# JuliaLinearAlgebra/AlgebraicMultigrid.jl

Measured on AMD Instinct MI355X. Metric: V-cycle unknowns/sec + fine-level SpMV GB/s (% HBM peak), 3-D Poisson 256^3, higher is better.
Workload: dtype f64

## Files before the change

### algebraicmultigrid.jl_amd/_libs.py

```python
import ctypes as C
import os

_HERE = os.path.dirname(os.path.abspath(__file__))
SETUP_SO = os.path.join(_HERE, "libamgsetup.so")
HIP_SO = os.path.join(_HERE, "libamghip.so")
HIP_F32_SO = os.path.join(_HERE, "libamghip_f32.so")

i32p = C.POINTER(C.c_int32)
f64p = C.POINTER(C.c_double)
i64 = C.c_int64
vp = C.c_void_p


class AMGError(RuntimeError):
    pass


class amgs_options(C.Structure):
    _fields_ = [("theta", C.c_double), ("max_levels", C.c_int32), ("max_coarse", C.c_int32),
                ("hermitian", C.c_int32), ("sa_omega", C.c_double), ("sa_improve_iters", C.c_int32),
                ("sa_B_is_vector", C.c_int32)]


class amgh_smoother_t(C.Structure):
# ... 141 lines not shown
    L.amgh_dev_upload.argtypes = [C.c_int, vp, vp, i64]
    L.amgh_dev_download.argtypes = [C.c_int, vp, vp, i64]
    L.amgh_dev_sync.argtypes = [C.c_int]
    L.amgh_stream.restype = vp
    L.amgh_stream.argtypes = [vp]
    L.amgh_timer_begin.argtypes = [vp]
    L.amgh_timer_end.argtypes = [vp, C.POINTER(C.c_double)]
    L.amgh_bench_op.argtypes = [vp, C.c_int, C.c_int, C.c_int, C.c_int, C.POINTER(C.c_double)]
    L.amgh_debug_chain_timing.argtypes = [C.c_int, vp]
    L.amgh_debug_merged_sweep_host.argtypes = [i64, i64, vp, vp, vp, C.c_int, C.c_int, C.c_double, vp, vp]
    L.amgh_debug_bw_poll_giveups.argtypes = [vp, C.c_int]
    L.amgh_debug_bw_mode.argtypes = [vp, C.c_int]
    L.amgh_debug_bw_dict.argtypes = [vp, C.c_int]
    L.amgh_debug_bw_late.argtypes = [vp, C.c_int]
    L.amgh_debug_coded_ops.argtypes = [vp, C.c_int]
    L.amgh_debug_bw_sweep_host.argtypes = [i64, vp, vp, vp, C.c_int, C.c_int, C.c_double, vp, vp, vp]
    L.amgh_debug_bw_dict_sweep_host.argtypes = [i64, vp, vp, vp, C.c_int, C.c_int, vp, vp, vp]
    L.amgh_debug_set_tunable.argtypes = [C.c_char_p, C.c_int]
    L.amgh_debug_get_tunable.argtypes = [C.c_char_p, C.POINTER(C.c_int)]
    L.amgh_profile_enable.argtypes = [vp, C.c_int]
    L.amgh_profile_read.argtypes = [vp, vp, C.c_int]
    L.amgh_set_use_graph.argtypes = [vp, C.c_int]


def _bind_dist(L):
    i64p = C.POINTER(i64)
    L.amgh_dist_rccl_available.argtypes = []
    L.amgh_dist_unique_id.argtypes = [vp]
    L.amgh_dist_create_rccl.argtypes = [C.POINTER(vp), C.c_int, C.c_int, C.c_int, vp]
    L.amgh_local_group_create.argtypes = [C.POINTER(vp), C.c_int]
# ... 100 lines not shown
```

### algebraicmultigrid.jl_amd/csrc/hip/amghip.hip

```cpp
#include "amghip_internal.hpp"
#include "gs_schedule.hpp"
#include "csr_ops.hpp"
#include "chebyshev.hpp"
#include "gmres_kernels.hpp"
#include "pcg_block_kernels.hpp"

namespace {

constexpr int64_t kGraphAutoRows = 65536;

struct Level {
  int64_t n = 0, nc = 0;
  amgh_csr A, S, P, R;
  bool has_S = false;
  amgh_smoother_t pre{}, post{};
  real *res = nullptr, *cx = nullptr, *cb = nullptr, *tmp = nullptr;
  real* cheb_d = nullptr;
  ChebSide cheb[2];
  const ChebSide& cheb_of(const amgh_smoother_t& s) const { return &s == &post ? cheb[1] : cheb[0]; }
  real* il = nullptr;
  amgh_csr* smat() { return has_S ? &S : &A; }
  amgh_csr Pp, Rp;
  bool lo_ok = false;
  real* lo_val = nullptr;
// ... 112 lines not shown
  if (n <= 0) return AMGH_OK;
  if (h->coarse_fn) {
    HIP_TRY(hipMemcpyAsync(h->coarse_hb.data(), b, sizeof(real) * n, hipMemcpyDeviceToHost, h->stream));
    HIP_TRY(hipStreamSynchronize(h->stream));
    if (h->coarse_fn(h->coarse_user, h->coarse_hb.data(), h->coarse_hx.data(), n) != 0) return AMGH_ESTATE;
    HIP_TRY(hipMemcpyAsync(x, h->coarse_hx.data(), sizeof(real) * n, hipMemcpyHostToDevice, h->stream));
    HIP_TRY(hipStreamSynchronize(h->stream));
    return AMGH_OK;
  }
  hipLaunchKernelGGL(dense_gemv_kernel, dim3((n + 63) / 64), dim3(64), 0, h->stream, h->coarse_op, b, x, n);
  HIP_TRY(hipGetLastError());
  return AMGH_OK;
}

int smooth(amgh_t* h, Level* L, const amgh_smoother_t& s, real*& xc, real*& xo, const real* b, int ncolv = 1,
           bool xzero = false, bool reuse_b = false, bool x_resident = false, bool no_scatter = false) {
  amgh_csr* M = L->smat();
  for (int it = 0; it < s.iter; ++it) {
    switch (s.kind) {
      case AMGH_SMOOTH_NONE: break;
      case AMGH_SMOOTH_JACOBI:
        if (xzero && it == 0 && g_jacobi_zero) RC_TRY(csr_jacobi_zero(M, s.omega, b, xo, h->stream, ncolv));
        else RC_TRY(csr_jacobi(M, s.omega, xc, b, xo, h->stream, ncolv));
        std::swap(xc, xo);
        break;
      case AMGH_SMOOTH_CHEBYSHEV: {
        const ChebSide& cs = L->cheb_of(s);
        if ((int)cs.c.size() != 2 * s.sweep || !L->cheb_d || !xo) return AMGH_ESTATE;
        for (int k = 0; k < s.sweep; ++k) {
          const real c1 = (real)cs.c[2 * (size_t)k], c2 = (real)cs.c[2 * (size_t)k + 1];
          if (k == 0 && xzero && it == 0 && g_jacobi_zero) RC_TRY(csr_chebyshev_zero(M, c2, b, L->cheb_d, xo, h->stream, ncolv));
          else RC_TRY(csr_chebyshev(M, c1, c2, k == 0, xc, b, L->cheb_d, xo, h->stream, ncolv));
          std::swap(xc, xo);
        }
        break;
      }
      case AMGH_SMOOTH_GS:
      case AMGH_SMOOTH_SOR: {
        const bool sor = s.kind == AMGH_SMOOTH_SOR;
        const bool sym = s.sweep == AMGH_SWEEP_SYMMETRIC;
        const bool first_it = (it == 0), last_it = (it == s.iter - 1);
        if (sym && M->gs && gs_wave_path(M->gs, sor)) {
          RC_TRY(csr_gs_sweep(M, false, sor, s.omega, xc, b, h->stream, first_it, last_it, ncolv, xzero && first_it,
                              reuse_b || !first_it, x_resident, no_scatter, true));
          break;
        }
        if (s.sweep == AMGH_SWEEP_FORWARD || sym)
          RC_TRY(csr_gs_sweep(M, false, sor, s.omega, xc, b, h->stream, first_it, last_it && !sym, ncolv, xzero && first_it,
                              reuse_b || !first_it, x_resident, no_scatter));
        if (s.sweep == AMGH_SWEEP_BACKWARD || sym)
          RC_TRY(csr_gs_sweep(M, true, sor, s.omega, xc, b, h->stream, first_it && !sym, last_it, ncolv,
                              xzero && first_it && !sym, reuse_b || !first_it, x_resident, no_scatter));
        break;
      }
      default: return AMGH_EINVAL;
    }
  }
  return AMGH_OK;
}

int cycle(amgh_t* h, int l, real* x, const real* b, int cyc, bool xzero, bool lo_io = false);

inline bool tail_here(const amgh_t* h, int l, int cyc) {
  return g_tail_dense && !h->tail_building && h->tail_level == l && cyc >= 0 && cyc < 3 && h->tail[cyc].built;
}
template <int NC, bool ACC>
int tail_launch(const real* M, int64_t n, real* x, int64_t ldx, const real* b, int64_t ldb, int groups, hipStream_t st) {
  if (n <= 1024) hipLaunchKernelGGL((dense_rm_gemv_kernel<NC, 64, ACC>), dim3((unsigned)n, groups), dim3(64), 0, st, M, b, x, (int)n, ldb, ldx);
  else hipLaunchKernelGGL((dense_rm_gemv_kernel<NC, 256, ACC>), dim3((unsigned)n, groups), dim3(256), 0, st, M, b, x, (int)n, ldb, ldx);
  HIP_TRY(hipGetLastError());
  return AMGH_OK;
}
template <bool ACC>
int tail_apply_t(amgh_t* h, const real* M, int64_t n, real* x, int64_t ldx, const real* b, int64_t ldb, int ncolv) {
  if (ncolv % 8 == 0) return tail_launch<8, ACC>(M, n, x, ldx, b, ldb, ncolv / 8, h->stream);
  if (ncolv % 4 == 0) return tail_launch<4, ACC>(M, n, x, ldx, b, ldb, ncolv / 4, h->stream);
  if (ncolv % 2 == 0) return tail_launch<2, ACC>(M, n, x, ldx, b, ldb, ncolv / 2, h->stream);
  return tail_launch<1, ACC>(M, n, x, ldx, b, ldb, ncolv, h->stream);
}
int tail_apply(amgh_t* h, const real* M, int64_t n, real* x, int64_t ldx, const real* b, int64_t ldb, int ncolv, bool acc) {
  return acc ? tail_apply_t<true>(h, M, n, x, ldx, b, ldb, ncolv) : tail_apply_t<false>(h, M, n, x, ldx, b, ldb, ncolv);
}

int cycle_next(amgh_t* h, int l, real* x, const real* b, int cyc, bool lo_io = false) {
  switch (cyc) {
    case AMGH_CYCLE_V: return cycle(h, l, x, b, AMGH_CYCLE_V, true, lo_io);
    case AMGH_CYCLE_W:
      RC_TRY(cycle(h, l, x, b, AMGH_CYCLE_W, true, lo_io));
      return cycle(h, l, x, b, AMGH_CYCLE_W, false, lo_io);
    case AMGH_CYCLE_F:
      RC_TRY(cycle(h, l, x, b, AMGH_CYCLE_F, true, lo_io));
      return cycle(h, l, x, b, AMGH_CYCLE_V, false, lo_io);
  }
  return AMGH_EINVAL;
}

int cycle(amgh_t* h, int l, real* x, const real* b, int cyc, bool xzero, bool lo_io) {
  Level* L = h->levels[l];
  const int bs = h->nrhs;
  const int64_t n = L->n, nc = L->nc;
  real* xc = x;
  real* xo = L->tmp;
  GsSchedule* g = L->smat()->gs;
  const bool lo = L->lo_ok && g && g->nblk == 0;
  if (lo_io && !lo) return AMGH_ESTATE;
  {
    ProfScope p(h, AMGH_T_PRESMOOTH, l);
    RC_TRY(smooth(h, L, L->pre, xc, xo, b, bs, xzero,  lo_io,  lo_io && !xzero,  lo));
  }
  if (lo) {
    Level* C = (L->coarse_lo && l + 1 < (int)h->levels.size()) ? h->levels[l + 1] : nullptr;
    GsSchedule* cg = C ? C->smat()->gs : nullptr;
    if (C && !(cg && C->lo_ok && cg->nblk == 0 && cg->cols_alloc >= bs)) return AMGH_ESTATE;
    const int64_t xs = g->xstride;
    {
      ProfScope p(h, AMGH_T_RESIDUAL, l);
      if (il_block(bs) && g_rhs_il >= 2)
        RC_TRY(resid_cols(bs, g->rowptr, g->col, L->lo_val ? L->lo_val : g->val, n, g->xp, xs, g->bp, n, L->res, n, h->stream, &L->lo_cc));
      else
        RC_TRY(raw_apply(M_RESID, g->rowptr, g->col, L->lo_val ? L->lo_val : g->val, n, g->xp, xs, g->bp, n, L->res, n,
                         h->stream, bs, &L->lo_cc));
    }
    {
      ProfScope p(h, AMGH_T_RESTRICT, l);
      if (L->il && il_block(bs) && !(L->r_stream && g_rhs_il == 1))
        RC_TRY(il_apply(bs, false, L->Rp.rowptr, L->Rp.col, L->Rp.val, nc, L->res, n, n, L->il, C ? cg->bp : L->cb, nc, h->stream, &L->Rp.cc));
      else
        RC_TRY(csr_apply(&L->Rp, M_SPMV, L->res, nullptr, C ? cg->bp : L->cb, h->stream, bs));
      if (C) cg->bp_cols = bs;
    }
    if (!C) RC_TRY(vec_fill(h, L->cx, nc * bs, 0.0));
    if (l == (int)h->levels.size() - 1) {
      ProfScope p(h, AMGH_T_COARSE, l + 1);
      for (int c = 0; c < bs; ++c) RC_TRY(coarse_solve(h, L->cx + c * nc, L->cb + c * nc));
    } else if (tail_here(h, l + 1, cyc) && (C != nullptr) == h->tail_lo) {
      ProfScope p(h, AMGH_T_COARSE, l + 1);
      RC_TRY(tail_apply(h, h->tail[cyc].M, nc, C ? cg->xp : L->cx, C ? cg->xstride : nc, C ? (const real*)cg->bp : (const real*)L->cb, nc, bs, false));
    } else {
      RC_TRY(cycle_next(h, l + 1, L->cx, L->cb, cyc, C != nullptr));
    }
    {
      ProfScope p(h, AMGH_T_PROLONG, l);
      if (L->il && il_block(bs) && !(L->p_stream && g_rhs_il == 1))
        RC_TRY(il_apply(bs, true, L->Pp.rowptr, L->Pp.col, L->Pp.val, n, C ? cg->xp : L->cx, nc, C ? cg->xstride : nc, L->il,
                        g->xp, xs, h->stream, &L->Pp.cc));
      else
        RC_TRY(raw_apply(M_ADD, L->Pp.rowptr, L->Pp.col, L->Pp.val, n, C ? cg->xp : L->cx, C ? cg->xstride : nc, nullptr, 0, g->xp,
                         xs, h->stream, bs, &L->Pp.cc));
    }
    {
      ProfScope p(h, AMGH_T_POSTSMOOTH, l);
      RC_TRY(smooth(h, L, L->post, xc, xo, b, bs, false, true, true,  lo_io));
    }
    return AMGH_OK;
// ... 2088 lines not shown
  else if (!strcmp(name, "gs_bigslot")) *value = g_gs_bigslot;
  else if (!strcmp(name, "gs_super")) *value = g_gs_super;
  else if (!strcmp(name, "gs_block_pipe")) *value = g_gs_block_pipe;
  else return AMGH_EINVAL;
  return AMGH_OK;
}

int amgh_debug_set_perm_io(int on) {
  g_gs_flow_perm_io = on != 0;
  ++g_sched_epoch;
  return AMGH_OK;
}
int amgh_debug_get_perm_io(void) { return g_gs_flow_perm_io; }
int amgh_debug_perm_io_sweeps(int which) { return (which == 0 || which == 1) ? (int)(g_perm_io_sweeps[which] & 0x7fffffffu) : -1; }

int amgh_debug_chain_timing(int enable, unsigned long long* out8) {
  if (enable && !g_chain_tim) {
    HIP_TRY(hipMalloc((void**)&g_chain_tim, 8 * sizeof(unsigned long long)));
    HIP_TRY(hipMemset(g_chain_tim, 0, 8 * sizeof(unsigned long long)));
  }
  if (out8 && g_chain_tim) {
    HIP_TRY(hipDeviceSynchronize());
    HIP_TRY(hipMemcpy(out8, g_chain_tim, 8 * sizeof(unsigned long long), hipMemcpyDeviceToHost));
    HIP_TRY(hipMemset(g_chain_tim, 0, 8 * sizeof(unsigned long long)));
  }
  if (!enable && g_chain_tim) { hipFree(g_chain_tim); g_chain_tim = nullptr; }
  return AMGH_OK;
}

int amgh_profile_enable(amgh_t* h, int on) {
// ... 27 lines not shown
```

### algebraicmultigrid.jl_amd/csrc/hip/amghip_internal.hpp

```cpp
#pragma once
#include "amghip_kernels.hpp"
#include "gs_blocks.hpp"
#include "gs_flow.hpp"

#include <algorithm>
#include <chrono>
#include <cmath>
#include <cstdio>
#include <cstring>
#include <atomic>
#include <mutex>
#include <string>
#include <system_error>
#include <thread>
#include <utility>
#include <vector>

#include "../../../include/amghip.h"

using namespace amgh;

#define HIP_TRY(expr)                                   \
  do {                                                  \
    hipError_t e_ = (expr);                             \
// ... 329 lines not shown
int g_gs_bw = 1;
int g_gs_bw_rows = 512;
int g_gs_bw_flow = 1;
int g_gs_bw_spin = 0;
int g_gs_bw_skip_pub = -1;
int g_gs_bw_nc = -1;
int g_gs_bw_nrhs = 1;
int g_gs_bw_chain = 1;
int g_stream_code = 1;
int g_trim_coded = 1;
int g_gs_bw_inorder = 0;
int g_gs_bw_dict = 1;
int g_gs_bw_relay = 3;
int g_gs_flow_xzero = 1;
int g_gs_flow_perm_io = 1;
unsigned int g_perm_io_sweeps[2] = {0, 0};
int g_gs_bw_two_min_rows = 200000;
int g_gs_sell = 1;
int g_gs_lean = -1;
int g_gs_ept = 0;
int g_gs_lpr = 0;
int g_gs_il = 1;
int g_pcg_fused = 1;
int g_tail_dense_rows = 6144;
int g_tail_dense = 1;
int g_gs_dense_blk = 4096;
int g_gs_dense_tri = 1;
int g_gs_block_inverse = 1;

std::atomic<unsigned long long> g_sched_epoch{0};
// ... 64 lines not shown
```

### algebraicmultigrid.jl_amd/csrc/hip/csr_ops.hpp

```cpp
#pragma once
#include <atomic>

namespace {


template <int MODE, class CFG = DefaultCfg, bool CODED = false>
int launch_stream(const StreamArgs& a0, hipStream_t st, int ncolv = 1) {
  const int nrows = a0.row_end - a0.row_begin;
  if (nrows <= 0) return AMGH_OK;
  StreamArgs a = a0;
  a.ncolv = ncolv;
  const int nb = (nrows + CFG::ROWS - 1) / CFG::ROWS;
  const int64_t grid = (CFG::XCD || ncolv > 1) ? (int64_t)((nb + kNumXcd - 1) / kNumXcd) * kNumXcd * ncolv : nb;
  hipLaunchKernelGGL((csr_stream_kernel<MODE, CFG, CODED>), dim3((unsigned)grid), dim3(CFG::THREADS), 0, st, a);
  HIP_TRY(hipGetLastError());
  return AMGH_OK;
}

constexpr int kGsBlockTarget = 256;
constexpr int kGsMinRows = 4;
constexpr int kGsNnzPerWg = 256;
template <int MODE>
int launch_gs_level(const StreamArgs& a, int rows, hipStream_t st, int ncolv = 1) {
  const int width = a.row_end - a.row_begin;
// ... 471 lines not shown
    if (hipMemset(fresh, 0, mb) != hipSuccess) { (void)hipGetLastError(); (void)hipFree(fresh); return -1001; }
    (void)hipFree(g->bw.flow.mbox);
    g->bw.flow.mbox = fresh;
    const int64_t more = g->bw.flow.mail_stride * (int64_t)(ncolv - g->bw.flow.mcols);
    g->bw.flow.bytes += more; g->bw.rec_bytes += more; g->slot_bytes += more;
    grown += more;
    g->bw.flow.mcols = ncolv;
  }
  g->bytes += grown;
  op->bytes += grown;
  g->cols_alloc = ncolv;
  g->bp_cols = 0;
  return AMGH_OK;
}

int csr_gs_sweep(amgh_csr* op, bool backward, bool sor, real omega, real* x, const real* b, hipStream_t st,
                 bool first = true, bool last = true, int ncolv = 1, bool xzero = false, bool reuse_b = false,
                 bool x_resident = false, bool no_scatter = false, bool sym_pair = false) {
  RC_TRY(csr_ensure_gs(op));
  GsSchedule* g = op->gs;
  if (g->n <= 0) return AMGH_OK;
  if (sym_pair && (backward || !gs_wave_path(g, sor))) return AMGH_EINVAL;
  RC_TRY(gs_ensure_cols(op, ncolv, st));
  if (g->dti_f && g_gs_dense_tri && g_gs_block_inverse && !sor) {
    g->bp_cols = 0;
    const GsSchedule::Tri& t = backward ? g->dtri_b : g->dtri_f;
    const int B = g->dti_B, nb = (int)g->dti_off.size() - 1;
    for (int q = 0; q < nb; ++q) {
      const int k = backward ? nb - 1 - q : q;
      const int r0 = k * B, rb = (int)std::min<int64_t>(B, g->n - r0);
      StreamArgs ra{};
      ra.rowptr = t.rowptr; ra.col = t.col; ra.val = t.val;
      ra.x = x; ra.b = b; ra.y = g->blk_s;
      ra.row_begin = r0; ra.row_end = r0 + rb;
      ra.ldx = g->n; ra.ldy = g->n; ra.ldb = g->n;
      if (nb > 1) RC_TRY((launch_stream<M_RESID, StreamCfg<256, 8, 4096, 2, false, false>>(ra, st, ncolv)));
      else RC_TRY((launch_stream<M_RESID, StreamCfg<256, 64, 4096, 2, false, false>>(ra, st, ncolv)));
      const real* Xk = (const real*)((backward ? g->dti_b : g->dti_f) + g->dti_off[k]);
// ... 70 lines not shown
    }
  }
  const int64_t xs = g->xstride;
  const bool il = g_gs_il && g_gs_lpr != 1 && lay != g && !g->bw.on && (ncolv == 8 || ncolv == 4 || ncolv == 2);
  if (first || !il) g->xil_cols = 0;
  bool il_s_ok = false;
  if (il && g->xil_cap < xs * ncolv) {
    HIP_TRY(hipStreamSynchronize(st));
    ++g_sched_epoch;
    hipFree(g->xil); g->xil = nullptr; g->xil_cap = 0;
    RC_TRY(dev_alloc(&g->xil, xs * ncolv));
    g->xil_cap = xs * ncolv;
    g->bytes += (int64_t)sizeof(real) * xs * ncolv; op->bytes += (int64_t)sizeof(real) * xs * ncolv;
    g->xil_cols = 0;
  }
  const bool perm_io = g_gs_flow_perm_io && ncolv == 1 && g->ncols == g->n && lay == g && !op->pipe_epoch && g_gs_bw_relay > 0 &&
                       g->bw.on && g->bw.flow.on && (g_gs_bw_flow || !g->bw.rec) &&
                       (int64_t)sizeof(real) * g->n < 0x7ffffff0ll;
  const bool fuse_b = perm_io && first && !(reuse_b && g->bp_cols == ncolv);
  const bool fuse_x = perm_io && last && !no_scatter && bw::relay_perm_x_ok<real>(g->bw.maxk, g->bw.flow.dict_on && (g_gs_bw_dict || !g->bw.flow.srec)) &&
                      ((g->bw.flow.dict_on && (g_gs_bw_dict || !g->bw.flow.srec)) ? g->bw.flow.dict_lds : g->bw.flow.lds_max) + bw::relay_perm_lds<real>(g->bw.flow.lds_max) <= 64 * 1024;
  if (first) {
    if (!(reuse_b && g->bp_cols == ncolv) && !fuse_b)
      hipLaunchKernelGGL(gather_perm_kernel, dim3(grid_for(g->n), ncolv), dim3(256), 0, st, b, g->perm, g->bp, (int)g->n,
                         (int64_t)g->n, (int64_t)g->n);
    g->bp_cols = ncolv;
    if (x_resident) {
    } else if (xzero) {
      const bool flow_zero = g_gs_flow_xzero && g->bw.on && g->bw.flow.on && (g_gs_bw_flow || !g->bw.rec) && g->ncols == g->n && lay == g;
      if (!flow_zero) {
        const int64_t cnt = xs * ncolv;
        hipLaunchKernelGGL(fill_kernel, dim3(grid_for(cnt)), dim3(256), 0, st, g->xp, cnt, 0.0);
        if (il) {
          const int64_t ci = g->ncols * ncolv;
          hipLaunchKernelGGL(fill_kernel, dim3(grid_for(ci)), dim3(256), 0, st, g->xil, ci, 0.0);
          g->xil_cols = ncolv;
// ... 71 lines not shown
      if (ncolv > g->bw.flow.mcols) return AMGH_ESTATE;
      const bool dict = g->bw.flow.dict_on && (g_gs_bw_dict || !g->bw.flow.srec);
      if (op->pipe_epoch) {
        if (ncolv != 1 || !g->bw.flow.xon) return AMGH_ESTATE;
        fa.aux = g->bw.flow.xaux; fa.fl_mb = g->bw.flow.xfl_mb; fa.fl_slot = g->bw.flow.xfl_slot; fa.xlist = g->bw.flow.xlist;
        fa.epoch = op->pipe_epoch; fa.rmbox = op->pipe_rmbox; fa.grid = op->pipe_grid;
        if (dict) { fa.crec = g->bw.flow.crec; fa.dict = g->bw.flow.dict; fa.dict_ent = g->bw.flow.dict_ent; }
        e = bw::sweep_relay<real>(fa, g->bw.maxk, dict ? g->bw.flow.dict_lds : g->bw.flow.lds_max, sor, backward, st, BW_RELAY_W);
      } else if (ncolv == 1 && g_gs_bw_relay > 0) {
        constexpr int kBwGrid = 0, kBwGridLong = 512;
        fa.grid = g->bw.maxk > 6 ? (dict ? 0 : kBwGridLong) : kBwGrid;
        fa.late = (g->bw.flow.late_ok && !g_gs_bw_inorder) ? 1 : 0;
        if (dict) { fa.crec = g->bw.flow.crec; fa.dict = g->bw.flow.dict; fa.dict_ent = g->bw.flow.dict_ent; }
        if (fuse_b) { fa.perm_b = g->perm; fa.b_nat = b; }
        if (fuse_x) { fa.perm_x = g->perm; fa.x_nat = x; }
        if (fuse_b || fuse_x) {
          e = bw::sweep_relay_io<real>(fa, g->bw.maxk, dict ? g->bw.flow.dict_lds : g->bw.flow.lds_max, g->bw.flow.lds_max, sor, backward, st);
          g_perm_io_sweeps[0] += fuse_b ? 1u : 0u; g_perm_io_sweeps[1] += fuse_x ? 1u : 0u;
        } else
        e = bw::sweep_relay<real>(fa, g->bw.maxk, dict ? g->bw.flow.dict_lds : g->bw.flow.lds_max, sor, backward, st, BW_RELAY_W);
      } else {
        if (dict) {
          fa.crec = g->bw.flow.crec; fa.dict = g->bw.flow.dict; fa.dict_ent = g->bw.flow.dict_ent;
          fa.dict_lds = (int32_t)(g->bw.flow.dict_lds - g->bw.flow.lds_max);
        }
        e = bw::sweep_flow<real>(fa, g->bw.maxk, g->bw.flow.lds_max, sor, backward, st, ncolv, g_gs_bw_nc >= 0 ? g_gs_bw_nc : (fa.crec ? 3 : 2));
      }
    } else {
      bw::Args<real> ba{g->bw.blocks, g->bw.rec, g->bw.ext_col, rhs, xp, ldb, xs, omega, 0, nullptr};
      if (g_gs_bw_chain && ncolv == 1 && g->bw.flags) {
        bw::ChainArgs<real> ca{ba, backward ? g->bw.sdep_ptr : g->bw.dep_ptr, backward ? g->bw.sdep : g->bw.dep, g->bw.flags, g->bw.head,
// ... 124 lines not shown
```

### algebraicmultigrid.jl_amd/csrc/hip/gs_flow.hpp

```cpp
#pragma once
#include "gs_blocks.hpp"

namespace amgh {
namespace bw {

constexpr int32_t kPubFwd = 1 << 30;
constexpr int32_t kPubBwd = (int32_t)(1u << 31);
constexpr int32_t kPubMask = (1 << 30) - 1;
#ifndef BW_FLOW_WAVES
#define BW_FLOW_WAVES 4
#endif
#ifndef BW_FLOW_DEPTH
#define BW_FLOW_DEPTH 4
#endif

struct FlowDesc {
  int32_t aux;
  int32_t npost;
  int32_t pad0, pad1;
};
constexpr int kStepRowBits = 11, kStepCntBits = 7, kStepNeedMax = (1 << 14) - 1;
inline uint32_t step_word(int r0, int nr, int need) { return (uint32_t)r0 | ((uint32_t)nr << kStepRowBits) | ((uint32_t)need << (kStepRowBits + kStepCntBits)); }

constexpr int32_t kRemoteCell = (int32_t)(1u << 31);
// ... 361 lines not shown
  unsigned int spin_limit;
  int32_t skip_pub;
  int64_t ldb = 0, ldx = 0, mail_stride = 0;
  int32_t lds_stride = 0;
  int32_t ncols = 1, ngroups = 1;
  int32_t xzero = 0;
  uint32_t epoch = 0;
  const unsigned char* crec = nullptr; const unsigned char* dict = nullptr; const int32_t* dict_ent = nullptr;
  int32_t dict_lds = 0;
  const int32_t* xlist = nullptr;
  const void* rmbox = nullptr;
  int32_t late = 0;
  int32_t grid = 0;
  const int32_t* perm_b = nullptr; const R* b_nat = nullptr;
  const int32_t* perm_x = nullptr; R* x_nat = nullptr;
};

template <typename R> struct Mail;
template <> struct Mail<double> {
  static constexpr int kBytes = 16;
  typedef u32x4 cell;
  static __device__ __forceinline__ cell load(__amdgpu_buffer_rsrc_t rs, unsigned off) { return __builtin_amdgcn_raw_buffer_load_b128(rs, off, 0, 16); }
  static __device__ __forceinline__ cell load_sys(__amdgpu_buffer_rsrc_t rs, unsigned off) { return __builtin_amdgcn_raw_buffer_load_b128(rs, off, 0, 17); }
  static __device__ __forceinline__ void store(__amdgpu_buffer_rsrc_t rs, unsigned off, double v, unsigned epoch) {
    const unsigned long long u = (unsigned long long)__double_as_longlong(v);
    cell c; c.x = (unsigned)u; c.y = epoch; c.z = (unsigned)(u >> 32); c.w = epoch;
    __builtin_amdgcn_raw_buffer_store_b128(c, rs, off, 0, 16);
  }
  static __device__ __forceinline__ bool valid(const cell& c, unsigned epoch) { return c.y == epoch && c.w == epoch; }
  static __device__ __forceinline__ double value(const cell& c) { return __longlong_as_double((long long)(((unsigned long long)c.z << 32) | c.x)); }
// ... 533 lines not shown
```

### algebraicmultigrid.jl_amd/csrc/hip/gs_relay.hpp

```cpp
#pragma once
#include "gs_flow.hpp"

namespace amgh {
namespace bw {

#ifndef BW_RELAY_W
#define BW_RELAY_W 3
#endif

#ifndef BW_RELAY_SPIN
#define BW_RELAY_SPIN 48u
#endif
#ifndef BW_RELAY_DEPTH_SHORT
#define BW_RELAY_DEPTH_SHORT 3
#endif
#ifndef BW_RELAY_DEPTH_LONG
#define BW_RELAY_DEPTH_LONG 2
#endif
template <int MAXK> struct RelayDepth { static constexpr int value = MAXK <= 12 ? BW_RELAY_DEPTH_SHORT : BW_RELAY_DEPTH_LONG; };
#ifndef BW_RELAY_FETCH_SLEEP
#define BW_RELAY_FETCH_SLEEP 4
#endif
#ifndef BW_RELAY_FETCH_PD
#define BW_RELAY_FETCH_PD 1
#endif
#ifndef BW_RELAY_FETCH_GAP
#define BW_RELAY_FETCH_GAP 6
#endif
#ifndef BW_RELAY_DICT_DEPTH
#define BW_RELAY_DICT_DEPTH 3
#endif
template <int MAXK> struct RelayDepthD { static constexpr int value = BW_RELAY_DICT_DEPTH; };
template <int MAXK> struct RelayWaves { static constexpr int value = MAXK <= 6 ? 4 : MAXK <= 18 ? 2 : 1; };
template <int MAXK> struct RelayWavesD { static constexpr int value = MAXK <= 6 ? 5 : MAXK <= 18 ? 3 : 2; };

template <typename T> __device__ __forceinline__ T lds_get(unsigned addr) { return *(const __attribute__((address_space(3))) T*)(unsigned long long)addr; }
template <typename T> __device__ __forceinline__ void lds_put(unsigned addr, T v) { *(__attribute__((address_space(3))) T*)(unsigned long long)addr = v; }
__device__ __forceinline__ unsigned lds_addr(const void* p) { return (unsigned)(unsigned long long)(const __attribute__((address_space(3))) unsigned char*)p; }

template <typename R, bool SOR, bool BWD, int MAXK, int W, bool DICT, bool LATE, bool PB, bool PX>
__device__ __forceinline__ void relay_block(const FlowArgs<R>& a, unsigned char* lds_all, const int wv, const int lane, const unsigned int ut,
                                            const unsigned int epoch, const long long t_start) {
  typedef typename std::conditional<DICT, FlowOpsD<R, MAXK>, FlowOps<R, MAXK>>::type O;
  typedef Mail<R> M;
  constexpr int D = DICT ? RelayDepthD<MAXK>::value : RelayDepth<MAXK>::value;
  constexpr int RB = (int)sizeof(R);
  constexpr int NVC = FlowOps<R, MAXK>::NVC;
  const bool fetcher = wv == W;
  const int tk = (int)ut;
  const int ob = __builtin_amdgcn_readfirstlane(BWD ? a.nblocks - 1 - tk : tk);
  const Desc d = a.blocks[ob];
  const FlowDesc f = a.fd[ob];
  const int ns = d.nlev;
  const int nxb = (int)(((size_t)(d.nrows + d.next + 1) * sizeof(R) + 15) & ~(size_t)15);
  const unsigned spin_limit = a.spin_limit ? a.spin_limit : (1u << 22);
// ... 241 lines not shown
          const int r0 = (int)(w & ((1u << kStepRowBits) - 1)), nr = (int)((w >> kStepRowBits) & ((1u << kStepCntBits) - 1));
          on[k] = lane < nr;
          pr[k] = on[k] ? r0 + lane : 0;
          pi[k] = pm[pr[k]];
        }
#pragma unroll
        for (int k = 0; k < SB; ++k) pin(pi[k]);
#pragma unroll
        for (int k = 0; k < SB; ++k) bv[k] = bn[pi[k]];
#pragma unroll
        for (int k = 0; k < SB; ++k) pin(bv[k]);
#pragma unroll
        for (int k = 0; k < SB; ++k) if (on[k]) bl[pr[k]] = bv[k];
      }
    }
    asm volatile("s_waitcnt vmcnt(0)" ::: "memory");
#pragma unroll
    for (int j = 0; j < D; ++j) issue(ops[j], wv + j * W);
  }
  __syncthreads();
  __builtin_amdgcn_s_setprio(2);
  const long long t_loaded = a.tim ? wall_clock64() : 0;
  const int32_t pubdir = BWD ? kPubBwd : kPubFwd;
  const bool mute = a.skip_pub == tk;
  const unsigned spare = (unsigned)a.nmail + (unsigned)(ob & 1023);
  bool gave_up = false, bail = false;
  const unsigned xl_base = (unsigned)__builtin_amdgcn_readfirstlane((int)lds_addr(xl));
  const unsigned ctl_off = xl_base + (unsigned)nxb;
  const unsigned dict_base = ctl_off + 16u;
  const unsigned perm_base = xl_base + (unsigned)__builtin_amdgcn_readfirstlane(perm_off);
#ifdef BW_RELAY_STAMPS
  const unsigned stamp_base = xl_base + (unsigned)nxb + 16u;
  i32x4 rs_pub = make_rsrc(a.tim + 4 * (int64_t)a.nblocks + 384 * (int64_t)a.nblocks);
  if (!a.tim) rs_pub.z = 0;
#endif
// ... 232 lines not shown
#endif
  if (a.tim && lane == 0) {
    long long* tt = a.tim + 4 * (int64_t)ob;
    if (wv == 0) {
      tt[0] = t_start; tt[1] = t_loaded;
      unsigned xcc = 0;
#ifdef BW_RELAY_STAMPS
      asm volatile("s_getreg_b32 %0, hwreg(HW_REG_XCC_ID)" : "=s"(xcc));
#endif
      tt[3] = (long long)(xcc & 15u);
    }
    if (wv == (ns - 1) % W) tt[2] = wall_clock64();
  }
}

template <typename R, bool SOR, bool BWD, int MAXK, int W, bool DICT = false, bool LATE = false, bool PB = false, bool PX = false>
__global__ __launch_bounds__(64 * (W + 1), DICT ? RelayWavesD<MAXK>::value : RelayWaves<MAXK>::value) void gs_bw_relay_kernel(FlowArgs<R> a) {
  extern __shared__ __attribute__((aligned(16))) unsigned char lds_all[];
  static_assert(W >= 2 && W <= 7, "walker waves per block");
#ifdef BW_RELAY_STAMPS
  static_assert(!PX, "the stamps of a measurement build lie where the slice of the permutation goes");
#endif
  const int wv = __builtin_amdgcn_readfirstlane((int)(threadIdx.x >> 6));
  const int lane = (int)(threadIdx.x & 63u);
  const unsigned int units = (unsigned int)a.nblocks;
  const bool persistent = gridDim.x < units;
  const unsigned int draws = units + (persistent ? gridDim.x : 0u);
  unsigned long long* s_ticket = (unsigned long long*)lds_all;
  if (blockIdx.x < 2048u) for (unsigned i = 0; i < (blockIdx.x >> 5); ++i) __builtin_amdgcn_s_sleep(14);
  for (;;) {
    const long long t_start = a.tim ? wall_clock64() : 0;
    if (threadIdx.x == 0) *s_ticket = atomicAdd(a.head, 1ull);
    __syncthreads();
    const unsigned long long tv = *s_ticket;
    const unsigned long long ticket = ((unsigned long long)(unsigned)__builtin_amdgcn_readfirstlane((int)(tv >> 32)) << 32) | (unsigned)__builtin_amdgcn_readfirstlane((int)tv);
    __syncthreads();
    const unsigned int ut = (unsigned int)ticket, sweeps = (unsigned int)(ticket >> 32);
    if (threadIdx.x == 0 && ut == draws - 1u)
      __hip_atomic_store(a.head, (unsigned long long)(sweeps + 2u >= 0x80000000u ? 0u : sweeps + 1u) << 32, __ATOMIC_RELAXED, __HIP_MEMORY_SCOPE_AGENT);
    if (ut >= units) return;
    const unsigned int epoch = a.epoch ? a.epoch : sweeps + 1u;
    relay_block<R, SOR, BWD, MAXK, W, DICT, LATE, PB, PX>(a, lds_all, wv, lane, ut, epoch, t_start);
    if (!persistent) return;
    __syncthreads();
  }
}
static_assert(RelayDepth<6>::value <= 4 && RelayDepth<12>::value <= 4 && RelayDepth<18>::value <= 4, "the first round of the relay's pipeline is written out for up to four sets");

inline size_t& relay_lds_pad() { static size_t pad = 0; return pad; }

template <typename R> inline size_t relay_perm_lds(size_t lds_x) {
  static_assert(sizeof(R) == 4 || sizeof(R) == 8, "4 bytes a row out of sizeof(R) bytes a row");
  return ((sizeof(R) == 8 ? (lds_x + 1) / 2 : lds_x) + 15) & ~(size_t)15;
}
template <typename R, bool SOR, bool BWD, int MAXK, int W, bool DICT = false, bool LATE = false, bool PB = false, bool PX = false>
inline hipError_t sweep_relay_launch(const FlowArgs<R>& a, size_t lds, hipStream_t st) {
  auto* fn = gs_bw_relay_kernel<R, SOR, BWD, MAXK, W, DICT, LATE, PB, PX>;
  if (relay_lds_pad()) {
    lds += relay_lds_pad();
    static hipError_t once = hipFuncSetAttribute((const void*)fn, hipFuncAttributeMaxDynamicSharedMemorySize, 160 * 1024);
    if (once != hipSuccess) return once;
    hipLaunchKernelGGL(fn, dim3((unsigned)(a.grid > 0 && a.grid < a.nblocks ? a.grid : a.nblocks)), dim3(64 * (W + 1)), lds, st, a);
    return hipGetLastError();
  }
#ifdef BW_RELAY_STAMPS
  lds += 128 * 24 + (DICT ? kDictLdsMax : 0);
#endif
  if (lds > 64 * 1024) return hipErrorInvalidValue;
  hipLaunchKernelGGL(fn, dim3((unsigned)(a.grid > 0 && a.grid < a.nblocks ? a.grid : a.nblocks)), dim3(64 * (W + 1)), lds, st, a);
  return hipGetLastError();
}
template <typename R, int MAXK, int W, bool DICT = false>
// ... 92 lines not shown
  if (px) return sweep_relay_io_k<R, MAXK, false, true>(a, lds, lds_x, sor, backward, st);
  return hipErrorInvalidValue;
}
template <typename R>
inline hipError_t sweep_relay_io(const FlowArgs<R>& a, int maxk, size_t lds_max, size_t lds_x, bool sor, bool backward, hipStream_t st) {
  switch (maxk) {
    case 6: return sweep_relay_io_m<R, 6>(a, lds_max, lds_x, sor, backward, st);
    case 12: return sweep_relay_io_m<R, 12>(a, lds_max, lds_x, sor, backward, st);
#if BW_PLAN_MAXK >= 18
    case 18: return sweep_relay_io_m<R, 18>(a, lds_max, lds_x, sor, backward, st);
#endif
  }
  return hipErrorInvalidValue;
}

}
}
```

### include/amghip.h

```cpp
#ifndef AMGHIP_H
#define AMGHIP_H

#include <stdint.h>

#ifdef __cplusplus
extern "C" {
#endif

#ifndef AMGH_REAL
#define AMGH_REAL double
#endif
typedef AMGH_REAL amgh_real;

typedef struct amgh_handle amgh_t;
typedef struct amgh_csr amgh_csr_t;

#define AMGH_OK 0
#define AMGH_EINVAL (-2)
#define AMGH_ESTATE (-3)
#define AMGH_ENOMEM (-4)
#define AMGH_EUNSUPPORTED (-5)

enum { AMGH_SMOOTH_NONE = 0, AMGH_SMOOTH_GS = 1, AMGH_SMOOTH_JACOBI = 2, AMGH_SMOOTH_SOR = 3, AMGH_SMOOTH_CHEBYSHEV = 4 };
enum { AMGH_SWEEP_FORWARD = 0, AMGH_SWEEP_BACKWARD = 1, AMGH_SWEEP_SYMMETRIC = 2 };
// ... 217 lines not shown
int amgh_debug_bw_dict_sweep_host(int64_t nrows, const int32_t* rowptr, const int32_t* col, const amgh_real* val, int target_rows,
                                  int backward, amgh_real* x, const amgh_real* b, int64_t* stats5);

int amgh_debug_bw_poll_giveups(const amgh_t* h, int l);

int amgh_debug_bw_mode(const amgh_t* h, int l);
int amgh_debug_bw_dict(const amgh_t* h, int l);
int amgh_debug_bw_late(const amgh_t* h, int l);
int amgh_debug_coded_ops(const amgh_t* h, int l);

int amgh_debug_set_tunable(const char* name, int value);
int amgh_debug_get_tunable(const char* name, int* value);
int amgh_debug_set_perm_io(int on);
int amgh_debug_get_perm_io(void);
int amgh_debug_perm_io_sweeps(int which);

int amgh_set_use_graph(amgh_t* h, int on);

#ifdef __cplusplus
}
#endif
#endif
```

Measured before the change: 1.211 billion.

## Fold restriction SpMV into the coarse level's first Gauss-Seidel relay sweep

When the next coarse level's pre-smoother is a Gauss-Seidel/SOR relay sweep in the permuted layout, the restriction R*res is no longer launched as its own SpMV. It is passed down as a SweepTransfer and computed inside the relay kernel's block-load phase, writing the permuted coarse RHS directly before the sweep starts. This removes one kernel launch and a separate pass over the coarse RHS per level. In exchange, each relay block does extra gather work before its dependency chain can begin, and the templated kernel variant gains more registers. It only applies to single-RHS, non-blocked schedules and is on by default.

```diff
diff --git a/algebraicmultigrid.jl_amd/_libs.py b/algebraicmultigrid.jl_amd/_libs.py
--- a/algebraicmultigrid.jl_amd/_libs.py
+++ b/algebraicmultigrid.jl_amd/_libs.py
@@ -179,6 +179,9 @@
     L.amgh_debug_bw_dict.argtypes = [vp, C.c_int]
     L.amgh_debug_bw_late.argtypes = [vp, C.c_int]
     L.amgh_debug_coded_ops.argtypes = [vp, C.c_int]
+    L.amgh_debug_set_transfer_io.argtypes = [C.c_int]
+    L.amgh_debug_get_transfer_io.argtypes = []
+    L.amgh_debug_transfer_io_sweeps.argtypes = [C.c_int]
     L.amgh_debug_bw_sweep_host.argtypes = [i64, vp, vp, vp, C.c_int, C.c_int, C.c_double, vp, vp, vp]
     L.amgh_debug_bw_dict_sweep_host.argtypes = [i64, vp, vp, vp, C.c_int, C.c_int, vp, vp, vp]
     L.amgh_debug_set_tunable.argtypes = [C.c_char_p, C.c_int]
diff --git a/algebraicmultigrid.jl_amd/csrc/hip/amghip.hip b/algebraicmultigrid.jl_amd/csrc/hip/amghip.hip
--- a/algebraicmultigrid.jl_amd/csrc/hip/amghip.hip
+++ b/algebraicmultigrid.jl_amd/csrc/hip/amghip.hip
@@ -150,8 +150,9 @@
 }
 
 int smooth(amgh_t* h, Level* L, const amgh_smoother_t& s, real*& xc, real*& xo, const real* b, int ncolv = 1,
-           bool xzero = false, bool reuse_b = false, bool x_resident = false, bool no_scatter = false) {
+           bool xzero = false, bool reuse_b = false, bool x_resident = false, bool no_scatter = false, const SweepTransfer* tr = nullptr) {
   amgh_csr* M = L->smat();
+  if (tr && !((s.kind == AMGH_SMOOTH_GS || s.kind == AMGH_SMOOTH_SOR) && s.iter > 0)) return AMGH_ESTATE;
   for (int it = 0; it < s.iter; ++it) {
     switch (s.kind) {
       case AMGH_SMOOTH_NONE: break;
@@ -178,15 +179,15 @@
         const bool first_it = (it == 0), last_it = (it == s.iter - 1);
         if (sym && M->gs && gs_wave_path(M->gs, sor)) {
           RC_TRY(csr_gs_sweep(M, false, sor, s.omega, xc, b, h->stream, first_it, last_it, ncolv, xzero && first_it,
-                              reuse_b || !first_it, x_resident, no_scatter, true));
+                              reuse_b || !first_it, x_resident, no_scatter, true, first_it ? tr : nullptr));
           break;
         }
         if (s.sweep == AMGH_SWEEP_FORWARD || sym)
           RC_TRY(csr_gs_sweep(M, false, sor, s.omega, xc, b, h->stream, first_it, last_it && !sym, ncolv, xzero && first_it,
-                              reuse_b || !first_it, x_resident, no_scatter));
+                              reuse_b || !first_it, x_resident, no_scatter, false, first_it ? tr : nullptr));
         if (s.sweep == AMGH_SWEEP_BACKWARD || sym)
           RC_TRY(csr_gs_sweep(M, true, sor, s.omega, xc, b, h->stream, first_it && !sym, last_it, ncolv,
-                              xzero && first_it && !sym, reuse_b || !first_it, x_resident, no_scatter));
+                              xzero && first_it && !sym, reuse_b || !first_it, x_resident, no_scatter, false, (first_it && !sym) ? tr : nullptr));
         break;
       }
       default: return AMGH_EINVAL;
@@ -195,7 +196,7 @@
   return AMGH_OK;
 }
 
-int cycle(amgh_t* h, int l, real* x, const real* b, int cyc, bool xzero, bool lo_io = false);
+int cycle(amgh_t* h, int l, real* x, const real* b, int cyc, bool xzero, bool lo_io = false, const SweepTransfer* tr = nullptr);
 
 inline bool tail_here(const amgh_t* h, int l, int cyc) {
   return g_tail_dense && !h->tail_building && h->tail_level == l && cyc >= 0 && cyc < 3 && h->tail[cyc].built;
@@ -218,20 +219,20 @@
   return acc ? tail_apply_t<true>(h, M, n, x, ldx, b, ldb, ncolv) : tail_apply_t<false>(h, M, n, x, ldx, b, ldb, ncolv);
 }
 
-int cycle_next(amgh_t* h, int l, real* x, const real* b, int cyc, bool lo_io = false) {
+int cycle_next(amgh_t* h, int l, real* x, const real* b, int cyc, bool lo_io = false, const SweepTransfer* tr = nullptr) {
   switch (cyc) {
-    case AMGH_CYCLE_V: return cycle(h, l, x, b, AMGH_CYCLE_V, true, lo_io);
+    case AMGH_CYCLE_V: return cycle(h, l, x, b, AMGH_CYCLE_V, true, lo_io, tr);
     case AMGH_CYCLE_W:
-      RC_TRY(cycle(h, l, x, b, AMGH_CYCLE_W, true, lo_io));
+      RC_TRY(cycle(h, l, x, b, AMGH_CYCLE_W, true, lo_io, tr));
       return cycle(h, l, x, b, AMGH_CYCLE_W, false, lo_io);
     case AMGH_CYCLE_F:
-      RC_TRY(cycle(h, l, x, b, AMGH_CYCLE_F, true, lo_io));
+      RC_TRY(cycle(h, l, x, b, AMGH_CYCLE_F, true, lo_io, tr));
       return cycle(h, l, x, b, AMGH_CYCLE_V, false, lo_io);
   }
   return AMGH_EINVAL;
 }
 
-int cycle(amgh_t* h, int l, real* x, const real* b, int cyc, bool xzero, bool lo_io) {
+int cycle(amgh_t* h, int l, real* x, const real* b, int cyc, bool xzero, bool lo_io, const SweepTransfer* tr) {
   Level* L = h->levels[l];
   const int bs = h->nrhs;
   const int64_t n = L->n, nc = L->nc;
@@ -240,9 +241,10 @@
   GsSchedule* g = L->smat()->gs;
   const bool lo = L->lo_ok && g && g->nblk == 0;
   if (lo_io && !lo) return AMGH_ESTATE;
+  if (tr && !lo_io) return AMGH_ESTATE;
   {
     ProfScope p(h, AMGH_T_PRESMOOTH, l);
-    RC_TRY(smooth(h, L, L->pre, xc, xo, b, bs, xzero,  lo_io,  lo_io && !xzero,  lo));
+    RC_TRY(smooth(h, L, L->pre, xc, xo, b, bs, xzero,  lo_io,  lo_io && !xzero,  lo, tr));
   }
   if (lo) {
     Level* C = (L->coarse_lo && l + 1 < (int)h->levels.size()) ? h->levels[l + 1] : nullptr;
@@ -257,7 +259,12 @@
         RC_TRY(raw_apply(M_RESID, g->rowptr, g->col, L->lo_val ? L->lo_val : g->val, n, g->xp, xs, g->bp, n, L->res, n,
                          h->stream, bs, &L->lo_cc));
     }
-    {
+    const bool next_cycles = l != (int)h->levels.size() - 1 && !(tail_here(h, l + 1, cyc) && (C != nullptr) == h->tail_lo);
+    const bool fold_r = C && next_cycles && bs == 1 && (C->pre.kind == AMGH_SMOOTH_GS || C->pre.kind == AMGH_SMOOTH_SOR) && C->pre.iter > 0 &&
+                        gs_transfer_fold_ok(C->smat(), 1, bs);
+    SweepTransfer rtr;
+    if (fold_r) { rtr.kind = 1; rtr.op = &L->Rp; rtr.src = L->res; rtr.ld = n; cg->bp_cols = bs; }
+    else {
       ProfScope p(h, AMGH_T_RESTRICT, l);
       if (L->il && il_block(bs) && !(L->r_stream && g_rhs_il == 1))
         RC_TRY(il_apply(bs, false, L->Rp.rowptr, L->Rp.col, L->Rp.val, nc, L->res, n, n, L->il, C ? cg->bp : L->cb, nc, h->stream, &L->Rp.cc));
@@ -273,7 +280,7 @@
       ProfScope p(h, AMGH_T_COARSE, l + 1);
       RC_TRY(tail_apply(h, h->tail[cyc].M, nc, C ? cg->xp : L->cx, C ? cg->xstride : nc, C ? (const real*)cg->bp : (const real*)L->cb, nc, bs, false));
     } else {
-      RC_TRY(cycle_next(h, l + 1, L->cx, L->cb, cyc, C != nullptr));
+      RC_TRY(cycle_next(h, l + 1, L->cx, L->cb, cyc, C != nullptr, fold_r ? &rtr : nullptr));
     }
     {
       ProfScope p(h, AMGH_T_PROLONG, l);
@@ -2392,6 +2399,14 @@
 int amgh_debug_get_perm_io(void) { return g_gs_flow_perm_io; }
 int amgh_debug_perm_io_sweeps(int which) { return (which == 0 || which == 1) ? (int)(g_perm_io_sweeps[which] & 0x7fffffffu) : -1; }
 
+int amgh_debug_set_transfer_io(int mask) {
+  g_gs_transfer_io = mask & 1;
+  ++g_sched_epoch;
+  return AMGH_OK;
+}
+int amgh_debug_get_transfer_io(void) { return g_gs_transfer_io; }
+int amgh_debug_transfer_io_sweeps(int which) { return (which == 0 || which == 1) ? (int)(g_transfer_io_sweeps[which] & 0x7fffffffu) : -1; }
+
 int amgh_debug_chain_timing(int enable, unsigned long long* out8) {
   if (enable && !g_chain_tim) {
     HIP_TRY(hipMalloc((void**)&g_chain_tim, 8 * sizeof(unsigned long long)));
diff --git a/algebraicmultigrid.jl_amd/csrc/hip/amghip_internal.hpp b/algebraicmultigrid.jl_amd/csrc/hip/amghip_internal.hpp
--- a/algebraicmultigrid.jl_amd/csrc/hip/amghip_internal.hpp
+++ b/algebraicmultigrid.jl_amd/csrc/hip/amghip_internal.hpp
@@ -367,6 +367,9 @@
 int g_gs_bw_relay = 3;
 int g_gs_flow_xzero = 1;
 int g_gs_flow_perm_io = 1;
+int g_gs_transfer_io = 1;
+unsigned int g_transfer_io_sweeps[2] = {0, 0};
+struct SweepTransfer { int kind = 0; const amgh_csr* op = nullptr; const real* src = nullptr; int64_t ld = 0; };
 unsigned int g_perm_io_sweeps[2] = {0, 0};
 int g_gs_bw_two_min_rows = 200000;
 int g_gs_sell = 1;
diff --git a/algebraicmultigrid.jl_amd/csrc/hip/csr_ops.hpp b/algebraicmultigrid.jl_amd/csrc/hip/csr_ops.hpp
--- a/algebraicmultigrid.jl_amd/csrc/hip/csr_ops.hpp
+++ b/algebraicmultigrid.jl_amd/csrc/hip/csr_ops.hpp
@@ -509,14 +509,30 @@
   return AMGH_OK;
 }
 
+bool gs_transfer_fold_ok(const amgh_csr* op, int kind, int ncolv) {
+  const GsSchedule* g = op->gs;
+  return kind == 1 && (g_gs_transfer_io & 1) && g && ncolv == 1 && g->n > 0 && g->ncols == g->n && !op->pipe_epoch && g_gs_bw_relay > 0 &&
+         g->bw.on && g->bw.flow.on && (g_gs_bw_flow || !g->bw.rec) && !g->mf && !g->mb && g->nblk == 0 && !(g->dti_f && g_gs_dense_tri && g_gs_block_inverse) &&
+         bw::relay_transfer_ok<real>(g->bw.maxk, g->bw.flow.dict_on && (g_gs_bw_dict || !g->bw.flow.srec));
+}
+int gs_transfer_alone(const SweepTransfer& t, GsSchedule* g, hipStream_t st, int ncolv) {
+  if (t.kind != 1 || !t.op || !t.src) return AMGH_EINVAL;
+  return csr_apply(t.op, M_SPMV, t.src, nullptr, g->bp, st, ncolv);
+}
+
 int csr_gs_sweep(amgh_csr* op, bool backward, bool sor, real omega, real* x, const real* b, hipStream_t st,
                  bool first = true, bool last = true, int ncolv = 1, bool xzero = false, bool reuse_b = false,
-                 bool x_resident = false, bool no_scatter = false, bool sym_pair = false) {
+                 bool x_resident = false, bool no_scatter = false, bool sym_pair = false, const SweepTransfer* tr = nullptr) {
   RC_TRY(csr_ensure_gs(op));
   GsSchedule* g = op->gs;
   if (g->n <= 0) return AMGH_OK;
   if (sym_pair && (backward || !gs_wave_path(g, sor))) return AMGH_EINVAL;
   RC_TRY(gs_ensure_cols(op, ncolv, st));
+  if (tr && !(first && tr->kind == 1)) return AMGH_EINVAL;
+  if (tr && ((g->dti_f && g_gs_dense_tri && g_gs_block_inverse && !sor) || (g->nblk > 0 && g_gs_block_inverse && !sor))) {
+    RC_TRY(gs_transfer_alone(*tr, g, st, ncolv));
+    tr = nullptr;
+  }
   if (g->dti_f && g_gs_dense_tri && g_gs_block_inverse && !sor) {
     g->bp_cols = 0;
     const GsSchedule::Tri& t = backward ? g->dtri_b : g->dtri_f;
@@ -617,12 +633,16 @@
     g->bytes += (int64_t)sizeof(real) * xs * ncolv; op->bytes += (int64_t)sizeof(real) * xs * ncolv;
     g->xil_cols = 0;
   }
-  const bool perm_io = g_gs_flow_perm_io && ncolv == 1 && g->ncols == g->n && lay == g && !op->pipe_epoch && g_gs_bw_relay > 0 &&
-                       g->bw.on && g->bw.flow.on && (g_gs_bw_flow || !g->bw.rec) &&
-                       (int64_t)sizeof(real) * g->n < 0x7ffffff0ll;
+  const bool perm_io_shape = ncolv == 1 && g->ncols == g->n && lay == g && !op->pipe_epoch && g_gs_bw_relay > 0 &&
+                             g->bw.on && g->bw.flow.on && (g_gs_bw_flow || !g->bw.rec);
+  const bool perm_io = g_gs_flow_perm_io && perm_io_shape && (int64_t)sizeof(real) * g->n < 0x7ffffff0ll;
   const bool fuse_b = perm_io && first && !(reuse_b && g->bp_cols == ncolv);
   const bool fuse_x = perm_io && last && !no_scatter && bw::relay_perm_x_ok<real>(g->bw.maxk, g->bw.flow.dict_on && (g_gs_bw_dict || !g->bw.flow.srec)) &&
                       ((g->bw.flow.dict_on && (g_gs_bw_dict || !g->bw.flow.srec)) ? g->bw.flow.dict_lds : g->bw.flow.lds_max) + bw::relay_perm_lds<real>(g->bw.flow.lds_max) <= 64 * 1024;
+  const bool fuse_r = tr && perm_io_shape && gs_transfer_fold_ok(op, tr->kind, ncolv) && !fuse_b && !fuse_x &&
+                      (tr->op->cc.ccol && (g_stream_code || !tr->op->col) ? tr->op->cc.vtab != nullptr : (tr->op->col && tr->op->val)) &&
+                      tr->op->nrows == g->n;
+  if (tr && !fuse_r) RC_TRY(gs_transfer_alone(*tr, g, st, ncolv));
   if (first) {
     if (!(reuse_b && g->bp_cols == ncolv) && !fuse_b)
       hipLaunchKernelGGL(gather_perm_kernel, dim3(grid_for(g->n), ncolv), dim3(256), 0, st, b, g->perm, g->bp, (int)g->n,
@@ -724,7 +744,14 @@
         if (dict) { fa.crec = g->bw.flow.crec; fa.dict = g->bw.flow.dict; fa.dict_ent = g->bw.flow.dict_ent; }
         if (fuse_b) { fa.perm_b = g->perm; fa.b_nat = b; }
         if (fuse_x) { fa.perm_x = g->perm; fa.x_nat = x; }
-        if (fuse_b || fuse_x) {
+        if (fuse_r) {
+          const amgh_csr* T = tr->op;
+          const bool coded = T->cc.ccol && (g_stream_code || !T->col);
+          fa.tr_rowptr = T->rowptr; fa.tr_src = tr->src;
+          if (coded) { fa.tr_ccol = T->cc.ccol; fa.tr_vtab = T->cc.vtab; } else { fa.tr_col = T->col; fa.tr_val = T->val; }
+          e = bw::sweep_relay_tr<real>(fa, 1, g->bw.maxk, dict ? g->bw.flow.dict_lds : g->bw.flow.lds_max, sor, backward, st);
+          g_transfer_io_sweeps[0] += 1u;
+        } else if (fuse_b || fuse_x) {
           e = bw::sweep_relay_io<real>(fa, g->bw.maxk, dict ? g->bw.flow.dict_lds : g->bw.flow.lds_max, g->bw.flow.lds_max, sor, backward, st);
           g_perm_io_sweeps[0] += fuse_b ? 1u : 0u; g_perm_io_sweeps[1] += fuse_x ? 1u : 0u;
         } else
diff --git a/algebraicmultigrid.jl_amd/csrc/hip/gs_flow.hpp b/algebraicmultigrid.jl_amd/csrc/hip/gs_flow.hpp
--- a/algebraicmultigrid.jl_amd/csrc/hip/gs_flow.hpp
+++ b/algebraicmultigrid.jl_amd/csrc/hip/gs_flow.hpp
@@ -399,6 +399,8 @@
   int32_t grid = 0;
   const int32_t* perm_b = nullptr; const R* b_nat = nullptr;
   const int32_t* perm_x = nullptr; R* x_nat = nullptr;
+  const int32_t* tr_rowptr = nullptr; const int32_t* tr_col = nullptr; const R* tr_val = nullptr;
+  const uint32_t* tr_ccol = nullptr; const R* tr_vtab = nullptr; const R* tr_src = nullptr;
 };
 
 template <typename R> struct Mail;
diff --git a/algebraicmultigrid.jl_amd/csrc/hip/gs_relay.hpp b/algebraicmultigrid.jl_amd/csrc/hip/gs_relay.hpp
--- a/algebraicmultigrid.jl_amd/csrc/hip/gs_relay.hpp
+++ b/algebraicmultigrid.jl_amd/csrc/hip/gs_relay.hpp
@@ -38,7 +38,7 @@
 template <typename T> __device__ __forceinline__ void lds_put(unsigned addr, T v) { *(__attribute__((address_space(3))) T*)(unsigned long long)addr = v; }
 __device__ __forceinline__ unsigned lds_addr(const void* p) { return (unsigned)(unsigned long long)(const __attribute__((address_space(3))) unsigned char*)p; }
 
-template <typename R, bool SOR, bool BWD, int MAXK, int W, bool DICT, bool LATE, bool PB, bool PX>
+template <typename R, bool SOR, bool BWD, int MAXK, int W, bool DICT, bool LATE, bool PB, bool PX, int TR>
 __device__ __forceinline__ void relay_block(const FlowArgs<R>& a, unsigned char* lds_all, const int wv, const int lane, const unsigned int ut,
                                             const unsigned int epoch, const long long t_start) {
   typedef typename std::conditional<DICT, FlowOpsD<R, MAXK>, FlowOps<R, MAXK>>::type O;
@@ -310,11 +310,86 @@
         for (int k = 0; k < SB; ++k) if (on[k]) bl[pr[k]] = bv[k];
       }
     }
+    if constexpr (TR == 1) {
+      constexpr int XR = 3, KU = 4;
+      const int32_t* rp = uniform_ptr(a.tr_rowptr) + d.row0;
+      const R* src = uniform_ptr(a.tr_src);
+      const uint32_t* tcc = uniform_ptr(a.tr_ccol);
+      const int32_t* tcl = uniform_ptr(a.tr_col);
+      const R* tvl = uniform_ptr(a.tr_val);
+      const R* tvt = uniform_ptr(a.tr_vtab);
+      R* bl = const_cast<R*>(a.b) + d.row0;
+      const bool coded = tcc != nullptr;
+      for (int p0 = wv * 64; p0 < d.nrows; p0 += 64 * W * XR) {
+        int32_t ks[XR], ke[XR]; R acc[XR];
+#pragma unroll
+        for (int q = 0; q < XR; ++q) {
+          const int p = p0 + lane + 64 * W * q;
+          ks[q] = rp[p < d.nrows ? p : 0];
+          ke[q] = rp[p < d.nrows ? p + 1 : 0];
+          acc[q] = (R)0;
+        }
+#pragma unroll
+        for (int q = 0; q < XR; ++q) { pin(ks[q]); pin(ke[q]); }
+        int len = 0;
+#pragma unroll
+        for (int q = 0; q < XR; ++q) len = ke[q] - ks[q] > len ? ke[q] - ks[q] : len;
+        for (int j0 = 0; __builtin_amdgcn_ballot_w64(j0 < len) != 0ull; j0 += KU) {
+          int32_t ci[XR][KU]; R tv[XR][KU], sv[XR][KU];
+          if (coded) {
+#pragma unroll
+            for (int q = 0; q < XR; ++q)
+#pragma unroll
+              for (int e = 0; e < KU; ++e) ci[q][e] = (int32_t)tcc[ks[q] + j0 + e < ke[q] ? ks[q] + j0 + e : 0];
+#pragma unroll
+            for (int q = 0; q < XR; ++q)
+#pragma unroll
+              for (int e = 0; e < KU; ++e) pin(ci[q][e]);
+#pragma unroll
+            for (int q = 0; q < XR; ++q)
+#pragma unroll
+              for (int e = 0; e < KU; ++e) { tv[q][e] = tvt[(unsigned)ci[q][e] >> 24]; sv[q][e] = src[(unsigned)ci[q][e] & 0xffffffu]; }
+          } else {
+#pragma unroll
+            for (int q = 0; q < XR; ++q)
+#pragma unroll
+              for (int e = 0; e < KU; ++e) {
+                const int kx = ks[q] + j0 + e < ke[q] ? ks[q] + j0 + e : 0;
+                ci[q][e] = tcl[kx]; tv[q][e] = tvl[kx];
+              }
+#pragma unroll
+            for (int q = 0; q < XR; ++q)
+#pragma unroll
+              for (int e = 0; e < KU; ++e) pin(ci[q][e]);
+#pragma unroll
+            for (int q = 0; q < XR; ++q)
+#pragma unroll
+              for (int e = 0; e < KU; ++e) sv[q][e] = src[ci[q][e]];
+          }
+#pragma unroll
+          for (int q = 0; q < XR; ++q)
+#pragma unroll
+            for (int e = 0; e < KU; ++e) {
+              R pr = tv[q][e] * sv[q][e];
+              pin(pr);
+              acc[q] = ks[q] + j0 + e < ke[q] ? acc[q] + pr : acc[q];
+            }
+        }
+#pragma unroll
+        for (int q = 0; q < XR; ++q) { const int p = p0 + lane + 64 * W * q; if (p < d.nrows) bl[p] = acc[q]; }
+      }
+    }
     asm volatile("s_waitcnt vmcnt(0)" ::: "memory");
+    if constexpr (TR != 1) {
+#pragma unroll
+      for (int j = 0; j < D; ++j) issue(ops[j], wv + j * W);
+    }
+  }
+  __syncthreads();
+  if constexpr (TR == 1) {
 #pragma unroll
     for (int j = 0; j < D; ++j) issue(ops[j], wv + j * W);
   }
-  __syncthreads();
   __builtin_amdgcn_s_setprio(2);
   const long long t_loaded = a.tim ? wall_clock64() : 0;
   const int32_t pubdir = BWD ? kPubBwd : kPubFwd;
@@ -577,10 +652,11 @@
   }
 }
 
-template <typename R, bool SOR, bool BWD, int MAXK, int W, bool DICT = false, bool LATE = false, bool PB = false, bool PX = false>
+template <typename R, bool SOR, bool BWD, int MAXK, int W, bool DICT = false, bool LATE = false, bool PB = false, bool PX = false, int TR = 0>
 __global__ __launch_bounds__(64 * (W + 1), DICT ? RelayWavesD<MAXK>::value : RelayWaves<MAXK>::value) void gs_bw_relay_kernel(FlowArgs<R> a) {
   extern __shared__ __attribute__((aligned(16))) unsigned char lds_all[];
   static_assert(W >= 2 && W <= 7, "walker waves per block");
+  static_assert(TR == 0 || (TR == 1 && !PB && !PX), "a grid transfer is folded into a sweep that folds no order change in");
 #ifdef BW_RELAY_STAMPS
   static_assert(!PX, "the stamps of a measurement build lie where the slice of the permutation goes");
 #endif
@@ -603,7 +679,7 @@
       __hip_atomic_store(a.head, (unsigned long long)(sweeps + 2u >= 0x80000000u ? 0u : sweeps + 1u) << 32, __ATOMIC_RELAXED, __HIP_MEMORY_SCOPE_AGENT);
     if (ut >= units) return;
     const unsigned int epoch = a.epoch ? a.epoch : sweeps + 1u;
-    relay_block<R, SOR, BWD, MAXK, W, DICT, LATE, PB, PX>(a, lds_all, wv, lane, ut, epoch, t_start);
+    relay_block<R, SOR, BWD, MAXK, W, DICT, LATE, PB, PX, TR>(a, lds_all, wv, lane, ut, epoch, t_start);
     if (!persistent) return;
     __syncthreads();
   }
@@ -616,9 +692,9 @@
   static_assert(sizeof(R) == 4 || sizeof(R) == 8, "4 bytes a row out of sizeof(R) bytes a row");
   return ((sizeof(R) == 8 ? (lds_x + 1) / 2 : lds_x) + 15) & ~(size_t)15;
 }
-template <typename R, bool SOR, bool BWD, int MAXK, int W, bool DICT = false, bool LATE = false, bool PB = false, bool PX = false>
+template <typename R, bool SOR, bool BWD, int MAXK, int W, bool DICT = false, bool LATE = false, bool PB = false, bool PX = false, int TR = 0>
 inline hipError_t sweep_relay_launch(const FlowArgs<R>& a, size_t lds, hipStream_t st) {
-  auto* fn = gs_bw_relay_kernel<R, SOR, BWD, MAXK, W, DICT, LATE, PB, PX>;
+  auto* fn = gs_bw_relay_kernel<R, SOR, BWD, MAXK, W, DICT, LATE, PB, PX, TR>;
   if (relay_lds_pad()) {
     lds += relay_lds_pad();
     static hipError_t once = hipFuncSetAttribute((const void*)fn, hipFuncAttributeMaxDynamicSharedMemorySize, 160 * 1024);
@@ -741,5 +817,38 @@
   return hipErrorInvalidValue;
 }
 
-}
-}
+
+template <typename R, int MAXK, bool DICT> struct RelayTransfer { static constexpr bool ok = MAXK > 12 || (sizeof(R) == 8 && (MAXK > 6 || !DICT)); };
+template <typename R> inline bool relay_transfer_ok(int maxk, bool dict) { return maxk > 12 || (sizeof(R) == 8 && (maxk > 6 || !dict)); }
+template <typename R, int MAXK, int TR>
+inline hipError_t sweep_relay_tr_k(const FlowArgs<R>& a0, size_t lds, bool sor, bool backward, hipStream_t st) {
+  constexpr int W = BW_RELAY_W;
+  FlowArgs<R> a = a0;
+  a.ncols = 1; a.ngroups = 1; a.lds_stride = 0;
+  auto go = [&](auto dict, auto late) -> hipError_t {
+    constexpr bool DC = decltype(dict)::value, LT = decltype(late)::value;
+    if constexpr (!RelayTransfer<R, MAXK, DC>::ok) return hipErrorInvalidValue;
+    else {
+      if (sor) return backward ? sweep_relay_launch<R, true, true, MAXK, W, DC, LT, false, false, TR>(a, lds, st) : sweep_relay_launch<R, true, false, MAXK, W, DC, LT, false, false, TR>(a, lds, st);
+      return backward ? sweep_relay_launch<R, false, true, MAXK, W, DC, LT, false, false, TR>(a, lds, st) : sweep_relay_launch<R, false, false, MAXK, W, DC, LT, false, false, TR>(a, lds, st);
+    }
+  };
+  if (a.crec) return a.late ? go(std::true_type(), std::true_type()) : go(std::true_type(), std::false_type());
+  return a.late ? go(std::false_type(), std::true_type()) : go(std::false_type(), std::false_type());
+}
+template <typename R>
+inline hipError_t sweep_relay_tr(const FlowArgs<R>& a, int tr, int maxk, size_t lds_max, bool sor, bool backward, hipStream_t st) {
+  if (tr != 1 || !a.tr_rowptr || !a.tr_src || !a.b || !(a.tr_ccol ? a.tr_vtab != nullptr : (a.tr_col && a.tr_val))) return hipErrorInvalidValue;
+  if (a.perm_b || a.perm_x) return hipErrorInvalidValue;
+  switch (maxk) {
+    case 6: return sweep_relay_tr_k<R, 6, 1>(a, lds_max, sor, backward, st);
+    case 12: return sweep_relay_tr_k<R, 12, 1>(a, lds_max, sor, backward, st);
+#if BW_PLAN_MAXK >= 18
+    case 18: return sweep_relay_tr_k<R, 18, 1>(a, lds_max, sor, backward, st);
+#endif
+  }
+  return hipErrorInvalidValue;
+}
+
+}
+}
diff --git a/include/amghip.h b/include/amghip.h
--- a/include/amghip.h
+++ b/include/amghip.h
@@ -255,6 +255,9 @@
 int amgh_debug_set_perm_io(int on);
 int amgh_debug_get_perm_io(void);
 int amgh_debug_perm_io_sweeps(int which);
+int amgh_debug_set_transfer_io(int mask);
+int amgh_debug_get_transfer_io(void);
+int amgh_debug_transfer_io_sweeps(int which);
 
 int amgh_set_use_graph(amgh_t* h, int on);
 
```

Result: no change. 1.216 billion, median of 6 (+0.4%).
